# ziqin-h/GIVEPose

Measured on AMD Instinct MI355X. Metric: images/sec PoseNet fwd, bs=64 256x256 fp16, 1/2/4/8 MI355X; % MFMA roofline, higher is better.
Workload: dtype f16

## Files before the change

givepose_amd/_lib.py:

```python
import ctypes
import os
from ctypes import POINTER, Structure, c_char_p, c_double, c_float, c_int, c_long, c_void_p

_HERE = os.path.dirname(os.path.abspath(__file__))
LIB_PATH = os.environ.get("GP_LIB_PATH") or os.path.join(_HERE, "libgivepose_hip.so")

ABI_VERSION = 328
GP_F32, GP_F16, GP_F64 = 0, 1, 2
ACT_NONE, ACT_GELU, ACT_RELU, ACT_LRELU = 0, 1, 2, 3
EPI_NONE, EPI_GELU, EPI_RELU, EPI_LRELU, EPI_SCALE_RES, EPI_RES_RELU, EPI_LNFOLD_GELU = 0, 1, 2, 3, 4, 5, 6
ROT_6D, ROT_6D_Y, ROT_6D_Z, ROT_QUAT, ROT_EULER = 0, 1, 2, 3, 4
KC_GEMM, KC_DCNV3, KC_DWCONV_LN, KC_NORM, KC_ELEMENTWISE, KC_SMALL, KC_COUNT = 0, 1, 2, 3, 4, 5, 6
KC_NAMES = ["gemm", "dcnv3", "dwconv_ln", "norm", "elementwise", "small"]


class GemmDesc(Structure):
    _fields_ = [("X", c_void_p), ("W", c_void_p), ("bias", c_void_p), ("gamma", c_void_p), ("residual", c_void_p),
                ("C", c_void_p), ("workspace", c_void_p),
                ("M", c_int), ("N", c_int), ("K", c_int), ("ldx", c_int), ("ldc", c_int), ("ldres", c_int),
                ("epilogue", c_int), ("out_f32", c_int), ("splitk", c_int),
                ("B", c_int), ("H", c_int), ("Win", c_int), ("Cin", c_int), ("KH", c_int), ("KW", c_int),
                ("stride", c_int), ("pad", c_int), ("Ho", c_int), ("Wo", c_int), ("dtype", c_int),
                ("gn_partial", c_void_p), ("gn_groups", c_int), ("gn_hw", c_int), ("variant", c_int),
                ("ln_stats", c_void_p), ("ln_colsum", c_void_p), ("ln_nslab", c_int), ("ln_eps", c_float),
# ... 316 lines not shown


class RepackBnFold(Structure):
    _fields_ = [(n, c_void_p) for n in ("w", "b", "bn_w", "bn_b", "mean", "var", "w_out", "b_out")] + [
        ("w_numel", c_longlong), ("c_numel", c_longlong), ("C", c_int), ("K", c_int), ("eps", c_float), ("pad", c_int)]


class RepackMatFold(Structure):
    _fields_ = [(n, c_void_p) for n in ("A", "B", "add", "out32", "out64")] + [
        (n, c_longlong) for n in ("a_numel", "b_numel", "add_numel", "out32_numel", "out64_numel")] + [
        (n, c_int) for n in ("M", "N", "K", "a_rs", "b_rs", "ld32", "ld64", "b_f64", "level", "pad")]


class RepackInfo(Structure):
    _fields_ = [(n, c_longlong) for n in ("bytes", "off_chunks", "off_bn", "off_mat", "off_mchunks")] + [
        (n, c_int) for n in ("n_entries", "n_chunks", "n_bn", "n_bn_blocks", "n_mat", "n_mchunks0", "n_mchunks1", "pad")]


REPACK_PROTOTYPES = {
    "gpr_tables_bytes": ([POINTER(RepackEntry), c_int, POINTER(RepackBnFold), c_int, POINTER(RepackMatFold), c_int], c_longlong),
    "gpr_tables_upload": ([POINTER(RepackEntry), c_int, POINTER(RepackBnFold), c_int, POINTER(RepackMatFold), c_int, _P, _P, c_longlong,
                           POINTER(RepackInfo), _P], c_int),
    "gpr_repack": ([_P, POINTER(RepackInfo), _P], c_int),
}
GPR_CHUNK, GPR_REPACK_LAUNCHES, GPR_REPACK_LAUNCHES_F32, GPR_MAX_ENTRIES, GPR_MAX_DIMS = 4096, 4, 3, 65536, 4
GPR_KIND_F32, GPR_KIND_F16, GPR_KIND_SPLIT = 0, 1, 2

TRAINDATA_PROTOTYPES = {
    "gpt_crop_train": ([_P] * 21 + [c_int] * 7 + [_P], c_int),
    "gpt_mask_deform": ([_P] * 3 + [c_ulonglong, _P, c_int, c_int, _P], c_int),
}
GPT_MAX_PIXELS, GPT_TRAIN_BATCH_LAUNCHES = 65536, 2

_lib = None


class GivePoseHipError(RuntimeError):
    pass


def load():
    global _lib
    if _lib is not None:
        return _lib
    if not os.path.exists(LIB_PATH):
        raise GivePoseHipError(
            f"{LIB_PATH} not found: build it with `python -m givepose_amd.build` (hipcc --offload-arch=gfx950). "
            "There is no CPU or PyTorch fallback for the product path.")
    lib = ctypes.CDLL(LIB_PATH)
    for name, (argtypes, restype) in (list(PROTOTYPES.items()) + list(ALIGN_PROTOTYPES.items()) + list(LOSS_PROTOTYPES.items())
                                      + list(GRAD_PROTOTYPES.items()) + list(HEADGRAD_PROTOTYPES.items())
                                      + list(XYZGRAD_PROTOTYPES.items()) + list(XYZGRAD_BF16_PROTOTYPES.items()) + list(ENCGRAD_PROTOTYPES.items())
                                      + list(ENCGRAD_ORDERED_PROTOTYPES.items())
                                      + list(BBGRAD_PROTOTYPES.items()) + list(BBGRAD_BF16_PROTOTYPES.items()) + list(OPTIM_PROTOTYPES.items())
                                      + list(SIZEGRAD_PROTOTYPES.items()) + list(ACCUM_PROTOTYPES.items())
                                      + list(REPACK_PROTOTYPES.items()) + list(TRAINDATA_PROTOTYPES.items())
                                      + list(ADAM_PROTOTYPES.items())):
        fn = getattr(lib, name)
        fn.argtypes = argtypes
        fn.restype = restype
    if lib.gp_version() != ABI_VERSION:
        raise GivePoseHipError(f"{LIB_PATH}: ABI version {lib.gp_version()}, this package needs {ABI_VERSION}: rebuild with "
                               "`python -m givepose_amd.build`")
    _lib = lib
    return lib


def check(rc, what=""):
    if rc != 0:
        msg = load().gp_last_error()
        raise GivePoseHipError(f"{what} failed ({rc}): {msg.decode() if msg else ''}")


_capturing = 0


def capturing():
    return _capturing > 0
```

givepose_amd/build.py:

```python
import os
import subprocess
import sys

HERE = os.path.dirname(os.path.abspath(__file__))
CSRC = os.path.join(HERE, "csrc")
OBJ = os.path.join(HERE, "csrc", "build")
LIB = os.path.join(HERE, "libgivepose_hip.so")
SOURCES = ["runtime.hip", "gemm.hip", "mlp.hip", "dcnv3.hip", "dcnv3_any.hip", "norm.hip", "misc.hip", "scalenet.hip", "evalmap.hip", "align.hip", "loss.hip", "lossgrad.hip", "pnpgrad.hip", "xyzgrad.hip", "encgrad.hip", "encscatter.hip", "bbgrad.hip", "optim.hip", "sizegrad.hip", "accum.hip", "repack.hip", "traindata.hip", "adam.hip"]
HIPCC = os.environ.get("HIPCC", "/opt/rocm/bin/hipcc")
FLAGS = ["-O3", "--offload-arch=gfx950", "-fPIC", "-std=c++17", "-Wno-unused-value"]
if os.environ.get("GP_PACKED_FP32") != "1":
    FLAGS += ["-Xclang", "-target-feature", "-Xclang", "-packed-fp32-ops", "-Wno-unknown-warning-option"]
EXTRA = os.environ.get("GP_EXTRA_HIPCC_FLAGS", "").split()
TAG = os.environ.get("GP_BUILD_TAG", "")
if EXTRA and not TAG:
    raise RuntimeError("GP_EXTRA_HIPCC_FLAGS needs GP_BUILD_TAG: an investigation build must not overwrite the product library")
if TAG:
    OBJ = os.path.join(HERE, "csrc", "build", "tag_" + TAG)
    LIB = os.path.join(HERE, f"libgivepose_hip_{TAG}.so")
    FLAGS += EXTRA


def _newer(a, b):
    return not os.path.exists(b) or os.path.getmtime(a) > os.path.getmtime(b)


def build(force=False, verbose=True):
    os.makedirs(OBJ, exist_ok=True)
    deps = [os.path.join(CSRC, "common.hpp"), os.path.join(HERE, "..", "include", "givepose_hip.h"),
            os.path.join(HERE, "..", "include", "givepose_align.h"), os.path.join(CSRC, "align_math.hpp"),
            os.path.join(HERE, "..", "include", "givepose_loss.h"), os.path.join(HERE, "..", "include", "givepose_grad.h"),
            os.path.join(HERE, "..", "include", "givepose_headgrad.h"), os.path.join(HERE, "..", "include", "givepose_xyzgrad.h"),
            os.path.join(HERE, "..", "include", "givepose_encgrad.h"), os.path.join(HERE, "..", "include", "givepose_bbgrad.h"),
            os.path.join(HERE, "..", "include", "givepose_optim.h"), os.path.join(HERE, "..", "include", "givepose_sizegrad.h"),
            os.path.join(HERE, "..", "include", "givepose_accum.h"), os.path.join(HERE, "..", "include", "givepose_repack.h"),
            os.path.join(HERE, "..", "include", "givepose_traindata.h"), os.path.join(CSRC, "grad_gemm.hpp"), os.path.join(CSRC, "grad_gemm_bf16.hpp"),
            os.path.join(HERE, "..", "include", "givepose_bbgrad_bf16.h"), os.path.join(CSRC, "xyz_conv_prec.hpp"),
            os.path.join(HERE, "..", "include", "givepose_xyzgrad_bf16.h"),
            os.path.join(HERE, "..", "include", "givepose_encgrad_ordered.h"), os.path.join(CSRC, "encscatter.hpp"),
            os.path.join(HERE, "..", "include", "givepose_adam.h")]
    objs, procs = [], []
    for src in SOURCES:
        s, o = os.path.join(CSRC, src), os.path.join(OBJ, src.replace(".hip", ".o"))
        objs.append(o)
        if force or _newer(s, o) or any(_newer(d, o) for d in deps):
            if verbose:
                print("hipcc", src, flush=True)
            procs.append((src, subprocess.Popen([HIPCC, *FLAGS, "-c", s, "-o", o])))
    for src, p in procs:
        if p.wait() != 0:
            raise RuntimeError(f"hipcc failed on {src}")
    if force or procs or not os.path.exists(LIB) or any(_newer(o, LIB) for o in objs):
        subprocess.check_call([HIPCC, "--offload-arch=gfx950", "-shared", "-fPIC", "-o", LIB, *objs])
        if verbose:
            print("linked", LIB)
    return LIB


if __name__ == "__main__":
    build(force="--force" in sys.argv)
```

givepose_amd/config.py:

```python
from dataclasses import dataclass, field
from typing import Tuple


ROT_TYPES = {
    "allo_rot6d": (6, 0, True), "ego_rot6d": (6, 0, False), "allo_rot6d_sym": (6, 0, True), "allo_rot6d_x": (6, 0, True),
    "allo_rot6d_sym_y": (6, 1, True), "allo_rot6d_y": (6, 1, True), "allo_rot6d_z": (6, 2, True),
    "allo_quat": (4, 3, True), "ego_quat": (4, 3, False), "euler": (6, 4, False),
}
FLAT_OPS = {"flatten": 0, "avg": 1, "avg-max": 2, "avg-max-min": 3}


def validate(cfg):
    def one_of(name, allowed):
        v = getattr(cfg, name)
        if v not in allowed:
            raise ValueError(f"{name}={v!r}: expected one of {sorted(allowed)}")
    if cfg.mask_attention_type == "concat":
        raise NotImplementedError("mask_attention_type='concat': the reference builds ConvPnPNet(5, ...) and then feeds it 6 channels "
                                  "(PoseNet.py:140,162; conv_pnp_net.py:73,152), so it cannot run this mode either")
    one_of("mask_attention_type", ("none", "mul"))
    one_of("flat_op", FLAT_OPS)
    one_of("r_type", ROT_TYPES)
    one_of("nocsmap_encoder", ("conv", "att"))
    one_of("use_dcn", ("dcnv3", ""))
# ... 11 lines not shown
                                      "its (B, 64, 192) tokens (attention_pnp_net.py:90-106), so fc1 gets 64 columns where it expects "
                                      f"{192 * FLAT_OPS[cfg.flat_op]}; the reference cannot run it either")
        if cfg.mask_attention_type == "mul":
            raise NotImplementedError("pnp_head='att' with mask_attention_type='mul': AttentionPnPNet.forward takes no mask "
                                      "(attention_pnp_net.py:121)")
        if ROT_TYPES[cfg.r_type][0] != 6:
            raise NotImplementedError(f"pnp_head='att' with r_type={cfg.r_type!r}: AttentionPnPNet's fc_r is Linear(256, 6) whatever the "
                                      "rotation type (attention_pnp_net.py:72), and a quaternion needs 4 outputs")


@dataclass(frozen=True)
class PoseNetConfig:
    main_backbone: str = "convnext"
    img_size: int = 256
    out_res: int = 64
    mask_attention_type: str = "none"
    feat_ts: int = 128
    flat_op: str = "flatten"
    t_type: str = "site"
    size_head_out_dim: int = 3
    nocsmap_encoder: str = "conv"
    r_type: str = "allo_rot6d"
    use_dcn: str = "dcnv3"
    dataset: str = "CAMERA+Real"
    convnext_dims: Tuple[int, ...] = (128, 256, 512, 1024)
    convnext_depths: Tuple[int, ...] = (3, 3, 27, 3)
    fuse_mlp: bool = True
    fuse_mlp_min_batch: int = 16
    defer_ln: bool = False

    res_fp32: bool = False
    deconv_cols_f16: bool = True
    gnxyz16: bool = True
    fuse_mlp512: bool = False
    pnp_head: str = "conv"

    @property
    def rot_dim(self) -> int:
        return ROT_TYPES[self.r_type][0] if self.r_type in ROT_TYPES else (4 if "quat" in self.r_type else 6)

    @property
    def fc_in_dim(self) -> int:
        k = FLAT_OPS[self.flat_op]
        if self.pnp_head == "att":
            return 192 * (k or 64)
        return 128 * (k or 64)

    @property
    def feature_channel(self) -> int:
        return {"convnext": self.convnext_dims[-1], "resnet34": 512}[self.main_backbone]
```

givepose_amd/csrc/misc.hip:

```cpp
#include "common.hpp"

namespace {

__device__ __forceinline__ void store_T(half_t* p, float v) { *p = (half_t)v; }
__device__ __forceinline__ void store_T(float* p, float v) { *p = v; }

template <typename T>
__global__ __launch_bounds__(256) void stem_kernel(const float* __restrict__ img, const float* __restrict__ wt,
                                                   const float* __restrict__ bias, const float* __restrict__ lnw,
                                                   const float* __restrict__ lnb, T* __restrict__ out, int H,
                                                   int W, float eps, int PXB) {
    constexpr int C0 = 128;
    __shared__ __attribute__((aligned(16))) float in_s[12][256];
    const int Ho = H / 4, Wo = W / 4;
    const int tid = threadIdx.x, lane = tid & 63, wave = tid >> 6;
    const int nwb = Wo / PXB;
    const int wblk = blockIdx.x % nwb;
    const int ho = (blockIdx.x / nwb) % Ho;
    const int b = blockIdx.x / (nwb * Ho);
    const int wo0 = wblk * PXB;
    for (int i = tid; i < 12 * PXB * 4; i += 256) {
        const int row = i / (PXB * 4), col = i - row * (PXB * 4);
        const int c = row >> 2, kh = row & 3;
        in_s[row][col] = img[(((long)b * 3 + c) * H + (ho * 4 + kh)) * W + wo0 * 4 + col];
    }
    float2 wr[48];
#pragma unroll
    for (int k = 0; k < 48; ++k) wr[k] = *reinterpret_cast<const float2*>(wt + k * C0 + lane * 2);
    const float2 bv = *reinterpret_cast<const float2*>(bias + lane * 2);
    const float2 gw = *reinterpret_cast<const float2*>(lnw + lane * 2), gb = *reinterpret_cast<const float2*>(lnb + lane * 2);
    __syncthreads();
    const int ppw = PXB / 4;
    for (int q = 0; q < ppw; ++q) {
// ... 283 lines not shown
template <typename T, typename CT>
__global__ __launch_bounds__(256) void col2im_kernel(const CT* __restrict__ cols, T* __restrict__ out, int B,
                                                     int H, int W, int C) {
    constexpr int VEC = 16 / sizeof(CT);
    const int CV = C / VEC, Ho = 2 * H, Wo = 2 * W;
    const long idx = (long)blockIdx.x * 256 + threadIdx.x;
    if (idx >= (long)B * Ho * Wo * CV) return;
    const int cv = (int)(idx % CV);
    long t = idx / CV;
    const int ox = (int)(t % Wo); t /= Wo;
    const int oy = (int)(t % Ho);
    const long b = t / Ho;
    float a[VEC];
#pragma unroll
    for (int e = 0; e < VEC; ++e) a[e] = 0.f;
    for (int ky = 0; ky < 3; ++ky) {
        const int ty = oy + 1 - ky;
        if (ty < 0 || (ty & 1)) continue;
        const int i = ty >> 1;
        if (i >= H) continue;
        for (int kx = 0; kx < 3; ++kx) {
            const int tx = ox + 1 - kx;
            if (tx < 0 || (tx & 1)) continue;
            const int j = tx >> 1;
            if (j >= W) continue;
            const Vec16<CT> v = load16<CT>(cols + ((b * H + i) * W + j) * (9L * C) + (ky * 3 + kx) * C + cv * VEC);
#pragma unroll
            for (int e = 0; e < VEC; ++e) a[e] += v.get(e);
        }
    }
    T* o = out + ((b * Ho + oy) * Wo + ox) * C + cv * VEC;
#pragma unroll
    for (int e = 0; e < VEC; ++e) store_T(o + e, a[e]);
}

template <typename T>
__global__ __launch_bounds__(256) void xyz_out_kernel(const T* __restrict__ x, const float* __restrict__ w,
                                                      const float* __restrict__ bias, float* __restrict__ out_nchw,
                                                      float* __restrict__ out_nhwc4, long rows, int HW, int C) {
    constexpr int VEC = Vec16<T>::N;
    const int chunks = C / VEC;
    const int LPP = chunks < 64 ? chunks : 64;
    const int lane = threadIdx.x & 63;
    const int sub = lane / LPP, l = lane % LPP;
    const int ppw = 64 / LPP;
    const long wave_id = (long)blockIdx.x * 4 + (threadIdx.x >> 6);
    const long row = wave_id * ppw + sub;
    float a0 = 0.f, a1 = 0.f, a2 = 0.f;
    if (row < rows) {
        for (int c = l; c < chunks; c += LPP) {
            const Vec16<T> v = load16<T>(x + row * C + c * VEC);
#pragma unroll
            for (int e = 0; e < VEC; ++e) {
                const float f = v.get(e);
                const int ch = c * VEC + e;
                a0 += f * w[ch];
                a1 += f * w[C + ch];
                a2 += f * w[2 * C + ch];
            }
        }
    }
    a0 = group_sum(a0, LPP); a1 = group_sum(a1, LPP); a2 = group_sum(a2, LPP);
    if (row < rows && l == 0) {
        a0 += bias[0]; a1 += bias[1]; a2 += bias[2];
        const long b = row / HW, pix = row - b * HW;
        out_nchw[(b * 3 + 0) * HW + pix] = a0;
// ... 638 lines not shown
               "gp_crop_rois: null pointer");
    GP_REQUIRE(B > 0 && B <= 65535 && F > 0 && NM > 0 && H > 0 && W > 0 && S > 0 && R > 0 && R <= S, "gp_crop_rois: bad shape");
    hipStream_t s = (hipStream_t)stream;
    gp_timing_before(s, GP_KC_SMALL, 0.0, (double)B * (S * S * 4.0 * 4 + S * S * 4.0 + R * R * 8.0));
    hipLaunchKernelGGL(crop_rois_kernel, dim3(cdiv(S * S, 256), B), dim3(256), 0, s, frames, masks, frame_idx, mask_idx, inv_img,
                       inv_out, img_lut, xlut, ylut, roi_img, roi_mask, roi_coord_2d, H, W, S, R);
    GP_LAUNCH_CHECK("gp_crop_rois");
}

extern "C" int gp_pred_rt(const float* R, const float* t, const float* size, const float* scale, float* pred_rt,
                          float* pred_size, int B, void* stream) {
    GP_REQUIRE(R && t && size && pred_rt && pred_size && B > 0, "gp_pred_rt: bad argument");
    hipStream_t s = (hipStream_t)stream;
    gp_timing_before(s, GP_KC_SMALL, 0.0, (double)B * 35 * 4);
    hipLaunchKernelGGL(pred_rt_kernel, dim3(cdiv(B, 64)), dim3(64), 0, s, R, t, size, scale, pred_rt, pred_size, B);
    GP_LAUNCH_CHECK("gp_pred_rt");
}

extern "C" int gp_deconv_col2im(const void* cols, void* out, int B, int H, int W, int C, int dtype_in, void* stream) {
    const int dtype = dtype_in & ~GP_COLS_F16;
    const bool c16 = (dtype_in & GP_COLS_F16) != 0;
    GP_REQUIRE(cols && out && B > 0 && C % (c16 ? 8 : 4) == 0, "gp_deconv_col2im: bad argument");
    GP_DT_OK(dtype);
    GP_REQUIRE(!c16 || dtype == GP_F16, "gp_deconv_col2im: fp16 cols go with fp16 output");
    hipStream_t s = (hipStream_t)stream;
    const long total = (long)B * 4 * H * W * (C / (c16 ? 8 : 4));
    gp_timing_before(s, GP_KC_ELEMENTWISE, (double)B * H * W * 9 * C, (double)B * H * W * 9 * C * (c16 ? 2 : 4) + (double)B * 4 * H * W * C * (dtype == GP_F16 ? 2 : 4));
    if (c16) hipLaunchKernelGGL((col2im_kernel<half_t, half_t>), dim3(cdiv(total, 256)), dim3(256), 0, s, (const half_t*)cols, (half_t*)out, B, H, W, C);
    else if (dtype == GP_F16) hipLaunchKernelGGL((col2im_kernel<half_t, float>), dim3(cdiv(total, 256)), dim3(256), 0, s, (const float*)cols, (half_t*)out, B, H, W, C);
    else hipLaunchKernelGGL((col2im_kernel<float, float>), dim3(cdiv(total, 256)), dim3(256), 0, s, (const float*)cols, (float*)out, B, H, W, C);
    GP_LAUNCH_CHECK("gp_deconv_col2im");
}

extern "C" int gp_xyz_out_layer(const void* x, const float* w, const float* b, float* out_nchw, float* out_nhwc4,
                                int B, int HW, int C, int dtype, void* stream) {
    GP_REQUIRE(x && w && b && out_nchw && out_nhwc4 && B > 0, "gp_xyz_out_layer: bad argument");
    GP_DT_OK(dtype);
    const int esz = dtype == GP_F16 ? 2 : 4, vec = 16 / esz, chunks = C / vec;
    GP_REQUIRE(C % vec == 0 && (chunks & (chunks - 1)) == 0, "gp_xyz_out_layer: C=%d", C);
    const int LPP = chunks < 64 ? chunks : 64, ppw = 64 / LPP;
    const long rows = (long)B * HW;
    hipStream_t s = (hipStream_t)stream;
    gp_timing_before(s, GP_KC_SMALL, 6.0 * rows * C, (double)rows * C * esz + rows * 28.0);
    dim3 grid(cdiv(rows, 4L * ppw));
    if (dtype == GP_F16) hipLaunchKernelGGL(xyz_out_kernel<half_t>, grid, dim3(256), 0, s, (const half_t*)x, w, b, out_nchw, out_nhwc4, rows, HW, C);
    else hipLaunchKernelGGL(xyz_out_kernel<float>, grid, dim3(256), 0, s, (const float*)x, w, b, out_nchw, out_nhwc4, rows, HW, C);
    GP_LAUNCH_CHECK("gp_xyz_out_layer");
}

extern "C" int gp_pointwise_k3(const float* xyz4, const float* w, const float* b, void* y, long rows, int Cout,
                               int dtype, void* stream) {
    GP_REQUIRE(xyz4 && w && b && y && rows > 0, "gp_pointwise_k3: bad argument");
    GP_DT_OK(dtype);
    const int esz = dtype == GP_F16 ? 2 : 4, vec = 16 / esz;
    GP_REQUIRE(Cout % vec == 0 && 256 % (Cout / vec) == 0, "gp_pointwise_k3: Cout=%d", Cout);
    hipStream_t s = (hipStream_t)stream;
    const long total = cdiv(rows, (256 / (Cout / vec)) * 8) * 256;
    gp_timing_before(s, GP_KC_ELEMENTWISE, 6.0 * rows * Cout, rows * 16.0 + (double)rows * Cout * esz);
    gp_timing_label("pointwise_k3 rows%ld Cout%d", rows, Cout);
    if (dtype == GP_F16) hipLaunchKernelGGL(pointwise_k3_kernel<half_t>, dim3(cdiv(total, 256)), dim3(256), 0, s, xyz4, w, b, (half_t*)y, rows, Cout);
    else hipLaunchKernelGGL(pointwise_k3_kernel<float>, dim3(cdiv(total, 256)), dim3(256), 0, s, xyz4, w, b, (float*)y, rows, Cout);
    GP_LAUNCH_CHECK("gp_pointwise_k3");
}

template <int CIN>
static int launch_smallcin(const float* xyz4, const float* coord2d, const float* w, void* y, int B, int R, int Cout,
// ... 236 lines not shown
```

givepose_amd/ops.py:

```python
import ctypes
import os

import torch

from . import _lib
from ._lib import (ACT_GELU, ACT_LRELU, ACT_NONE, ACT_RELU, EPI_GELU, EPI_LNFOLD_GELU, EPI_LRELU, EPI_NONE, EPI_RELU, EPI_RES_RELU,
                   EPI_SCALE_RES, GP_F16, GP_F32, GP_F64, GemmDesc, check)

__all__ = ["dtype_code", "gemm", "conv2d_nhwc", "dcnv3_forward", "dcnv3_backward", "dcnv3_forward_into", "dcnv3_xyz_project", "convnext_stem", "dwconv_ln",
           "layernorm", "groupnorm", "upsample_bilinear2x", "deconv_col2im", "xyz_out_layer", "pointwise_k3",
           "pnp_conv1", "pnp_conv1_masked", "pool_mmm", "xyz_conv3x3_s2", "size_head", "pose_tail", "pose_tail_rt", "mask_resize_nearest"]


def _L():
    return _lib.load()


def _stream():
    return ctypes.c_void_p(torch.cuda.current_stream().cuda_stream)


def dtype_code(dt):
    if dt == torch.float16:
        return GP_F16
    if dt == torch.float32:
        return GP_F32
    raise TypeError(f"unsupported dtype {dt} (float16 / float32)")


def _ptr(t):
    return None if t is None else ctypes.c_void_p(t.data_ptr())


def _chk(t, name, dtype=None):
    if not t.is_cuda:
        raise RuntimeError(f"{name} must be a CUDA tensor")
    if dtype is not None and t.dtype != dtype:
        raise TypeError(f"{name}: expected {dtype}, got {t.dtype}")
    return t


def _contig(t, name):
    if not t.is_contiguous():
# ... 400 lines not shown
    check(_L().gp_groupnorm_apply(_ptr(x), _ptr(partial), _ptr(w), _ptr(b), _ptr(out), B, HW, C, G, eps, act,
                                  C if ldy is None else ldy, HW // rows if fused_stats else 0, _planes_code(x, out_planes, out), _stream()),
          "gp_groupnorm_apply")
    return out


def groupnorm_upsample2x(x, w, b, out, G, act, partial, eps=1e-5, rows=64):
    B, H, W_, C = x.shape
    check(_L().gp_groupnorm_upsample2x(_ptr(_contig(x, "x")), _ptr(partial), _ptr(w), _ptr(b), _ptr(out), B, H, W_, C, G, eps, act,
                                       H * W_ // rows, dtype_code(x.dtype), _stream()), "gp_groupnorm_upsample2x")
    return out


def groupnorm_apply_xyz(x, w, b, out_w, out_b, out_nchw, out_nhwc4, G, act, partial, eps=1e-5, rows=64, packed16=False):
    B, HW, C = x.shape
    check(_L().gp_groupnorm_apply_xyz(_ptr(_contig(x, "x")), _ptr(partial), _ptr(w), _ptr(b), _ptr(out_w), _ptr(out_b),
                                      _ptr(out_nchw), _ptr(out_nhwc4), B, HW, C, G, eps, act | (0x100 if packed16 else 0), HW // rows, dtype_code(x.dtype),
                                      _stream()), "gp_groupnorm_apply_xyz")


def upsample_bilinear2x(x, out, out_planes=False):
    B, H, W_, C = x.shape
    check(_L().gp_upsample_bilinear2x(_ptr(_contig(x, "x")), _ptr(out), B, H, W_, C, _planes_code(x, out_planes, out), _stream()),
          "gp_upsample_bilinear2x")
    return out


def deconv_col2im(cols, out, B, H, W_, C):
    code = dtype_code(out.dtype) | (0x400 if cols.dtype == torch.float16 else 0)
    check(_L().gp_deconv_col2im(_ptr(cols), _ptr(out), B, H, W_, C, code, _stream()), "gp_deconv_col2im")
    return out


def xyz_out_layer(x, w, b, out_nchw, out_nhwc4):
    B, HW, C = x.shape
    check(_L().gp_xyz_out_layer(_ptr(_contig(x, "x")), _ptr(w), _ptr(b), _ptr(out_nchw), _ptr(out_nhwc4), B, HW, C,
                                dtype_code(x.dtype), _stream()), "gp_xyz_out_layer")


def pointwise_k3(xyz4, w, b, out):
    rows = xyz4.shape[0]
    check(_L().gp_pointwise_k3(_ptr(xyz4), _ptr(w), _ptr(b), _ptr(out), rows, w.shape[0], dtype_code(out.dtype), _stream()),
          "gp_pointwise_k3")
    return out


def dcnv3_xyz_project(xyz4, om, m, bias, out, gn, mask_col=72, mask_is_logits=True):
    _contig(_chk(xyz4, "xyz4"), "xyz4"), _contig(_chk(om, "om"), "om"), _contig(_chk(out, "out"), "out")
    rows = out.shape[0]
    if xyz4.dtype != torch.float32 or om.dtype != torch.float32 or m.dtype != torch.float32 or bias.dtype != torch.float32:
        raise TypeError("dcnv3_xyz_project: xyz4, om, m and bias are float32")
    if tuple(m.shape) != (256, 16) or bias.numel() != 256 or out.shape[1] != 256 or om.shape[0] < rows or xyz4.shape[0] < (rows + 1023) // 1024 * 4096:
        raise RuntimeError("dcnv3_xyz_project: shapes")
    if gn[0].numel() < (rows + 1023) // 1024 * 32 * 32 * 2:
        raise RuntimeError("dcnv3_xyz_project: the gn_partial buffer is too small for 32 chunks of 32 groups per crop")
    check(_L().gp_dcnv3_xyz_project(_ptr(xyz4), _ptr(om), _ptr(_contig(m, "m")), _ptr(bias), _ptr(out), _ptr(gn[0]), rows, 64, 64, 3, 2, 1, 1, 4,
                                    om.shape[1], mask_col, 1 if mask_is_logits else 0, gn[1], gn[2], gn[3], dtype_code(out.dtype), _stream()),
          "gp_dcnv3_xyz_project")
    return out


def pnp_conv1(xyz4, coord2d, w, out, B, R):
    check(_L().gp_pnp_conv1(_ptr(xyz4), _ptr(_contig(coord2d, "coord2d")), _ptr(w), _ptr(out), B, R, w.shape[1],
                            dtype_code(out.dtype), _stream()), "gp_pnp_conv1")
    return out

# ... 65 lines not shown
```

givepose_amd/posenet.py:

```python
import ctypes
import functools
import os
from collections import OrderedDict

import numpy as np
import torch
import torch.nn as nn

from . import _lib, ops, synth
from ._lib import (ACT_GELU, ACT_RELU, EPI_GELU, EPI_LNFOLD_GELU, EPI_LRELU, EPI_NONE, EPI_SCALE_RES)
from .config import FLAT_OPS, ROT_TYPES, PoseNetConfig, validate

OM_LD = 128


def enc0_xyz_pack(sd, prefix="nocs_encoder.features.0.", dtype=torch.float32):
    f64 = lambda k: sd[prefix + k].detach().to(device="cpu", dtype=torch.float64)
    cw, cb = f64("conv.weight").reshape(256, -1), f64("conv.bias")
    iw, ib = f64("dcnv3.input_proj.weight"), f64("dcnv3.input_proj.bias")
    ow, ob = f64("dcnv3.output_proj.weight"), f64("dcnv3.output_proj.bias")
    fold = torch.cat([iw @ cw, (iw @ cb + ib)[:, None]], 1)
    m = torch.cat([ow[:, 64 * g:64 * g + 64] @ fold[64 * g:64 * g + 64] for g in range(4)], 1)
    return m.to(dtype).contiguous(), ob.to(dtype).contiguous()

# ... 384 lines not shown
                buf[f"dsn{s}"] = e(B, h * 2, h * 2, dims[s - 1])
        buf["cols"] = e(B * 64, 9 * 256) if (T == torch.float16 and cfg.deconv_cols_f16 and os.environ.get("GP_DECONV_COLS_F32") != "1") else f(B * 64, 9 * 256)
        for r in (16, 32, 64):
            buf[f"ya{r}"], buf[f"yb{r}"] = e(B, r, r, 256), e(B, r, r, 256)
        chunks = max(ops.groupnorm_chunks(B, r * r) for r in (8, 16, 32, 64))
        buf["gn_partial"], buf["size_scratch"] = f(B * max(chunks, R * R // 16) * 32 * 2), f(B * (cfg.feat_ts + (512 if cfg.main_backbone == "resnet34" else cfg.convnext_dims[-1])))
        buf["nocs_nchw"], buf["nocs_nhwc4"] = f(B, 3, R, R), f(B * R * R, 4)
        buf["ivfc_nchw"], buf["ivfc_nhwc4"] = f(B, 3, R, R), f(B * R * R, 4)
        buf["mask_out"], buf["size"] = f(B, 1, R, R), f(B, 3)
        enc0_xyz = "enc0.xyz_m" in self._packed and os.environ.get("GP_ENC0_XYZ") != "0"
        for li, r in enumerate((64, 32, 16)):
            buf[f"e_in{li}"], buf[f"e_x1{li}"] = e(B, r, r, 256), e(B * r * r // 4, 256)
            buf[f"e_om{li}"] = f(B * r * r // 4, OM_LD)
            buf[f"e_o{li}"] = e(B, r // 2, r // 2, 256)
            if li > 0 or not enc0_xyz:
                buf[f"e_proj{li}"], buf[f"e_g{li}"] = e(B, r, r, 256), e(B, r // 2, r // 2, 256)
        if cfg.nocsmap_encoder == "att":
            buf["a_patch"], buf["a_x"], buf["a_h"] = e(B * 64, 192), e(B * 64, 256), e(B * 64, 256)
            buf["a_qkv"], buf["a_att"], buf["a_mlp"] = e(B * 64, 768), e(B * 64, 256), e(B * 64, 1024)
            buf["a_pos"] = self._packed["att.pos"].to(T).repeat(B, 1).contiguous()
        buf["feat_cat"] = e(B, 8, 8, 512)
        if cfg.pnp_head == "att":
            buf["p_patch"], buf["p_x"], buf["p_h"] = e(B * 64, 320), e(B * 64, 192), e(B * 64, 192)
            buf["p_qkv"], buf["p_att"], buf["p_mlp"], buf["p_flat"] = e(B * 64, 576), e(B * 64, 192), e(B * 64, 768), e(B * 64, 192)
            buf["p_pos"] = self._packed["apn.pos"].to(T).repeat(B, 1).contiguous()
        else:
            buf["p0"], buf["p1"], buf["p2"] = e(B, 32, 32, 128), e(B, 16, 16, 128), e(B, 8, 8, 128)
        buf["fc1"] = e(B, 2048)
        buf["hh"], buf["hz"] = f(B, 256), f(B, 256)
        if FLAT_OPS[cfg.flat_op]:
            buf["pooled"] = e(B, 128 * FLAT_OPS[cfg.flat_op])
        buf["pred_rot"], buf["pred_t"], buf["rot_allo"], buf["rot_ego"], buf["trans"] = f(B, cfg.rot_dim), f(B, 3), f(B, 9), f(B, 9), f(B, 3)
        buf["rot6d"] = buf["pred_rot"] if cfg.rot_dim == 6 else None
        plan = {"buf": buf, "graph": None, "warm": False, "ragged": bool(ragged), "enc0_xyz": enc0_xyz}
        if ragged:
            buf["grp"] = torch.arange(B, dtype=torch.int32, device=device)
            buf["grp_host"] = torch.arange(B, dtype=torch.int32).pin_memory()
            for k in ("roi_img", "roi_mask", "roi_coord_2d", "bbox_center", "mean_size"):
                buf[k].zero_()
            buf["roi_wh"].fill_(1.0)
            buf["resize_ratio"].fill_(1.0)
            buf["cam_K"].copy_(torch.eye(3, device=device).expand(B, 3, 3))
        self._plans[key] = plan
        self._evict_plans(key)
        return plan

    def _gn(self, x, w, b, act, buf, G=32, out=None, ldy=None, fused=False, out_planes=False, rows=64):
        B = x.shape[0]
        C = x.shape[-1]
        xv = x.view(B, -1, C)
        ops.groupnorm(xv, w, b, xv if out is None else out, G, act, buf["gn_partial"], ldy=ldy, fused_stats=fused, out_planes=out_planes, rows=rows)

    def _gnrows(self, M, N, K, hw):
        if self.split_gemm or self.compute_dtype != torch.float16 or os.environ.get("GP_GN_ROWS64") == "1":
            return 64
        return ops.gemm_gn_rows(M, N, K, hw)

    @staticmethod
    def _gnarg(buf, hw, rows=64):
        B = buf["mask_out"].shape[0]
        if B * (hw // rows) * 32 * 2 > buf["gn_partial"].numel():
            raise RuntimeError(f"fused GroupNorm statistics: {hw // rows} chunks of {rows} rows per image do not fit the plan's gn_partial buffer")
        return (buf["gn_partial"], 32, hw, rows)

    def _xyz_head(self, W, head, feat2d, B, buf, out_nchw, out_nhwc4):
        pl = self.split_gemm
        ops.gemm(feat2d, W[head + ".deconv_w"], buf["cols"], prefetch=W[f"{head}.c3_w"])
        y = ops.deconv_col2im(buf["cols"], buf["ya16"], B, 8, 8, 256)
        if pl:
            self._gn(y, W[head + ".gn0_w"], W[head + ".gn0_b"], ACT_GELU, buf, out=buf["yb16"].view(B, -1, 256), out_planes=True)
            y = buf["yb16"]
        else:
            self._gn(y, W[head + ".gn0_w"], W[head + ".gn0_b"], ACT_GELU, buf)
        cur, r = y, 16
        rows = {rr: self._gnrows(B * rr * rr, 256, 2304, rr * rr) for rr in (16, 32, 64)}
        fuse_up = FUSE_GN_UPSAMPLE and not pl and y.dtype == torch.float16
        for i in (3, 4, 6, 7, 9, 10):
            if i in (6, 9):
                r *= 2
                if fuse_up:
                    cur = ops.groupnorm_upsample2x(cur, W[f"{head}.c{i - 2}_gw"], W[f"{head}.c{i - 2}_gb"], buf[f"ya{r}"], 32, ACT_GELU,
                                                   buf["gn_partial"], rows=rows[r // 2])
                else:
                    cur = ops.upsample_bilinear2x(cur, buf[f"ya{r}"], out_planes=pl)
            dst = buf[f"yb{r}"] if cur is buf[f"ya{r}"] else buf[f"ya{r}"]
            nxt = {3: 4, 4: 6, 6: 7, 7: 9, 9: 10}.get(i)
            ops.conv2d_nhwc(cur, W[f"{head}.c{i}_w"], 3, 3, 1, 1, out=dst, gn=self._gnarg(buf, r * r, rows[r]),
                            prefetch=W[f"{head}.c{nxt}_w"] if nxt else None, x_planes=pl)
            if i == 10:
                ops.groupnorm_apply_xyz(dst.view(B, r * r, 256), W[f"{head}.c{i}_gw"], W[f"{head}.c{i}_gb"], W[head + ".out_w"],
                                        W[head + ".out_b"], out_nchw, out_nhwc4, 32, ACT_GELU, buf["gn_partial"], rows=rows[r],
                                        packed16=self.cfg.gnxyz16 and dst.dtype == torch.float16 and os.environ.get("GP_GNXYZ16") != "0")
            elif fuse_up and i in (4, 7):
                pass
            elif pl and i not in (4, 7):
                self._gn(dst, W[f"{head}.c{i}_gw"], W[f"{head}.c{i}_gb"], ACT_GELU, buf, fused=True, out=cur.view(B, -1, 256), out_planes=True, rows=rows[r])
                dst = cur
            else:
                self._gn(dst, W[f"{head}.c{i}_gw"], W[f"{head}.c{i}_gb"], ACT_GELU, buf, fused=True, rows=rows[r])
            cur = dst

    def _resnet34(self, W, buf):
        from ._lib import EPI_RELU, EPI_RES_RELU
        s = ops.resnet_stem(buf["roi_img"], W["rs.stem_w"], W["rs.stem_b"], buf["rs_stem"])
        x = ops.maxpool3x3s2(s, buf["rs1a"])
        for li, (planes, blocks, stride) in enumerate(synth.RESNET34_LAYERS, 1):
# ... 30 lines not shown
        for s, (d, n) in enumerate(zip(dims, depths)):
            if s > 0:
                t = ops.layernorm(x, W[f"ds{s}.ln_w"], W[f"ds{s}.ln_b"], buf[f"dsn{s}"], out_planes=self.split_gemm)
                x = ops.conv2d_nhwc(t, W[f"ds{s}.w"], 2, 2, 2, 0, out=buf[f"x{s}"], bias=W[f"ds{s}.b"], x_planes=self.split_gemm,
                                    out16=buf.get(f"x{s}h"))
            x2d = x.view(-1, d)
            xh = buf.get(f"x{s}h")
            xin = x if xh is None else xh
            for b in range(n):
                q = f"s{s}b{b}."
                if (q + "fc1_wg") in W and x2d.shape[0] % 256 == 0 and x.shape[1] % 4 == 0 and x.shape[2] % 16 == 0:
                    t = ops.dwconv7_raw_stats(x, W[q + "dw_w"], W[q + "dw_b"], buf[f"t{s}"], buf["ln_stats"])
                    ops.gemm(t.view(-1, d), W[q + "fc1_wg"], buf[f"h{s}"], bias=W[q + "fc1_cb"], epilogue=EPI_LNFOLD_GELU,
                             ln=(buf["ln_stats"], W[q + "fc1_cs"], d // 128, 1e-6))
                    ops.gemm(buf[f"h{s}"], W[q + "fc2_w"], x2d, bias=W[q + "fc2_b"], epilogue=EPI_SCALE_RES,
                             gamma=W[q + "gamma"], residual=x2d)
                    continue
                t = ops.dwconv_ln(xin, W[q + "dw_w"], W[q + "dw_b"], W[q + "ln_w"], W[q + "ln_b"], buf[f"t{s}"], 7, out_planes=self.split_gemm)
                if (q + "fc2_wp") in W and x2d.shape[0] % 256 == 0 and B >= cfg.fuse_mlp_min_batch and (d != 512 or x2d.shape[0] >= 32768):
                    ops.convnext_mlp(t.view(-1, d), W[q + "fc1_w"], W[q + "fc1_b"], W[q + "fc2_wp"], W[q + "fc2_b"],
                                     W[q + "gamma"], x2d, x2d)
                    continue
                pl = self.split_gemm
                ops.gemm(t.view(-1, d), W[q + "fc1_w"], buf[f"h{s}"], bias=W[q + "fc1_b"], epilogue=EPI_GELU, prefetch=W[q + "fc2_w"],
                         x_planes=pl, out_planes=pl)
                ops.gemm(buf[f"h{s}"], W[q + "fc2_w"], x2d, bias=W[q + "fc2_b"], epilogue=EPI_SCALE_RES,
                         gamma=W[q + "gamma"], residual=x2d, x_planes=pl, out16=None if xh is None else xh.view(-1, d),
                         prefetch=W.get(f"ds{s + 1}.w") if b == n - 1 else None)
        if cfg.main_backbone == "convnext":
            feat = x
        fc = dims[-1]
        feat2d = feat.view(B * 64, fc)
        ops.size_head(feat.view(B, 64, fc), W["size.w1"], W["size.b1"], W["size.w2"], W["size.b2"], buf["mean_size"], buf["size"], buf["size_scratch"])
        self._xyz_head(W, "xyz_nocs_head", feat2d, B, buf, buf["nocs_nchw"], buf["nocs_nhwc4"])
        self._seq_encoder(B, plan)
        cat2d = buf["feat_cat"].view(B * 64, 512)
        ops.gemm(feat2d, W["red.w"], cat2d, bias=W["red.b"], ldc=512)
        self._xyz_head(W, "xyz_deform_head", cat2d, B, buf, buf["ivfc_nchw"], buf["ivfc_nhwc4"])
        self._seq_pnp(B, plan)

    def _seq_encoder(self, B, plan, only_layer=None, weights_of=None):
        W, buf, cfg = self._packed, plan["buf"], self.cfg
        cat2d = buf["feat_cat"].view(B * 64, 512)
        prev = None
        if cfg.nocsmap_encoder == "att":
            x = buf["a_x"]
            ops.patchify_xyz(buf["nocs_nhwc4"], buf["a_patch"], B, cfg.out_res, 8)
            ops.gemm(buf["a_patch"], W["att.pe_w"], x, bias=W["att.pe_b"], epilogue=EPI_SCALE_RES, gamma=W["att.ones"],
                     residual=buf["a_pos"])
            for i in range(3):
                q = f"att{i}."
                h = ops.layernorm(x, W[q + "norm1_w"], W[q + "norm1_b"], buf["a_h"], eps=1e-5)
                ops.gemm(h, W[q + "qkv_w"], buf["a_qkv"])
                ops.attention64(buf["a_qkv"], buf["a_att"], B, 8)
                ops.gemm(buf["a_att"], W[q + "proj_w"], x, bias=W[q + "proj_b"], epilogue=EPI_SCALE_RES, gamma=W["att.ones"], residual=x)
                h = ops.layernorm(x, W[q + "norm2_w"], W[q + "norm2_b"], buf["a_h"], eps=1e-5)
                ops.gemm(h, W[q + "fc1_w"], buf["a_mlp"], bias=W[q + "fc1_b"], epilogue=EPI_GELU)
                ops.gemm(buf["a_mlp"], W[q + "fc2_w"], x, bias=W[q + "fc2_b"], epilogue=EPI_SCALE_RES, gamma=W["att.ones"], residual=x)
            ops.layernorm(x, W["att.norm_w"], W["att.norm_b"], cat2d[:, 256:], eps=1e-5, ldy=512)
        for li, r in enumerate((64, 32, 16) if cfg.nocsmap_encoder == "conv" else ()):
            q = f"enc{li}."
            ro = r // 2
            if only_layer is not None:
                if li != only_layer:
                    continue
                prev = buf[f"e_o{li - 1}"]
                if weights_of is not None:
                    q = f"enc{weights_of}."
            if cfg.use_dcn == "dcnv3":
                xin = buf[f"e_in{li}"]
                xyz0 = li == 0 and plan.get("enc0_xyz") and only_layer is None
# ... 186 lines not shown
                        _lib._capturing -= 1
                        ge = ctypes.c_void_p()
                        rc = lib.gp_graph_end(sp, ctypes.byref(ge))
                    _lib.check(rc, "gp_graph_end")
                    plan["graph"] = ge
                _lib.check(lib.gp_graph_launch(plan["graph"], sp), "gp_graph_launch")
            else:
                self._launch_all(B, plan)
                plan["warm"] = True
        if run_stream is not cur and wait:
            cur.wait_stream(run_stream)
        n = n_real
        feat = buf.get(f"x{len(self.cfg.convnext_dims) - 1}")
        return {"rot": buf["rot_ego"].view(B, 3, 3)[:n], "trans": buf["trans"][:n], "size": buf["size"][:n], "mask": buf["mask_out"][:n],
                "nocs_coor": buf["nocs_nchw"][:n], "ivfc_coor": buf["ivfc_nchw"][:n], "rot6d": None if buf["rot6d"] is None else buf["rot6d"][:n],
                "pred_rot": buf["pred_rot"][:n], "pred_t": buf["pred_t"][:n],
                "rot_allo": buf["rot_allo"].view(B, 3, 3)[:n], "feat": None if feat is None else feat[:n],
                "feat_cat": buf["feat_cat"][:n]}

    def _module_plan(self, B, device):
        device = torch.device(device)
        _lib.load()
        if self._packed is None:
            self._pack(device)
        return self._plan(B, device, 0)

    @torch.no_grad()
    def run_xyz_head(self, head, feat_nchw, device="cuda"):
        B, C = feat_nchw.shape[:2]
        plan = self._module_plan(B, device)
        buf = plan["buf"]
        x = feat_nchw.to(device).permute(0, 2, 3, 1).reshape(B * 64, C).to(self.compute_dtype).contiguous()
        key = "nocs" if head == "xyz_nocs_head" else "ivfc"
        self._xyz_head(self._packed, head, x, B, buf, buf[key + "_nchw"], buf[key + "_nhwc4"])
        return buf[key + "_nchw"].clone()

    @torch.no_grad()
    def run_map_encoder(self, coor_nchw, device="cuda"):
        B = coor_nchw.shape[0]
        plan = self._module_plan(B, device)
        buf = plan["buf"]
        buf["nocs_nhwc4"].zero_()
        buf["nocs_nhwc4"][:, :3] = coor_nchw.to(device).float().permute(0, 2, 3, 1).reshape(-1, 3)
        self._seq_encoder(B, plan)
        return buf["feat_cat"].view(B, 8, 8, 512)[..., 256:].permute(0, 3, 1, 2).float().contiguous()

    @torch.no_grad()
    def run_dcnv3_c(self, layer, x_nchw, device="cuda", weights_of=None):
        assert self.cfg.use_dcn == "dcnv3" and layer in (1, 2) and weights_of in (None, 1, 2)
        B = x_nchw.shape[0]
        plan = self._module_plan(B, device)
        buf = plan["buf"]
        buf[f"e_o{layer - 1}"].copy_(x_nchw.to(device).permute(0, 2, 3, 1).to(self.compute_dtype))
        self._seq_encoder(B, plan, only_layer=layer, weights_of=weights_of)
        return buf[f"e_o{layer}"].permute(0, 3, 1, 2).float().contiguous()

    @torch.no_grad()
    def run_pnp(self, x_nchw, data, device="cuda", mask=None):
        B = x_nchw.shape[0]
        if self.cfg.mask_attention_type == "mul" and mask is None:
            raise ValueError("run_pnp: mask_attention_type='mul' needs the (B,1,64,64) mask")
        plan = self._module_plan(B, device)
        buf = plan["buf"]
        if mask is not None:
            buf["mask_out"].copy_(mask.reshape(buf["mask_out"].shape))
        for k in ("cam_K", "roi_wh", "bbox_center", "resize_ratio"):
            buf[k].copy_(data[k].reshape(buf[k].shape))
# ... 373 lines not shown
```

Baseline: 12730.

## Fuse deconv col2im with GroupNorm and GELU in xyz heads

Adds a HIP kernel that performs the transposed-conv col2im gather for the first 16x16 map of each xyz head and computes GroupNorm statistics, affine and GELU inside one workgroup per image and channel slab. Each thread keeps its gathered pixels in registers for the two-pass mean and variance. This removes the intermediate ya16 write/read and the separate GroupNorm statistics and apply launches. The path is on by default for fp16, non-split plans and has an environment switch. The cost is a per-thread register footprint of GS half8 vectors and fixed shape requirements: a 256-pixel output map and 8 channels per group.

```diff
diff --git a/givepose_amd/_lib.py b/givepose_amd/_lib.py
--- a/givepose_amd/_lib.py
+++ b/givepose_amd/_lib.py
@@ -372,6 +372,10 @@
 }
 GPT_MAX_PIXELS, GPT_TRAIN_BATCH_LAUNCHES = 65536, 2
 
+FUSED_PROTOTYPES = {
+    "gpfu_deconv_col2im_gn": ([_P] * 4 + [c_int] * 5 + [c_float] + [c_int] * 2 + [_P], c_int),
+}
+
 _lib = None
 
 
@@ -395,7 +399,7 @@
                                       + list(BBGRAD_PROTOTYPES.items()) + list(BBGRAD_BF16_PROTOTYPES.items()) + list(OPTIM_PROTOTYPES.items())
                                       + list(SIZEGRAD_PROTOTYPES.items()) + list(ACCUM_PROTOTYPES.items())
                                       + list(REPACK_PROTOTYPES.items()) + list(TRAINDATA_PROTOTYPES.items())
-                                      + list(ADAM_PROTOTYPES.items())):
+                                      + list(ADAM_PROTOTYPES.items()) + list(FUSED_PROTOTYPES.items())):
         fn = getattr(lib, name)
         fn.argtypes = argtypes
         fn.restype = restype
diff --git a/givepose_amd/build.py b/givepose_amd/build.py
--- a/givepose_amd/build.py
+++ b/givepose_amd/build.py
@@ -38,7 +38,7 @@
             os.path.join(HERE, "..", "include", "givepose_bbgrad_bf16.h"), os.path.join(CSRC, "xyz_conv_prec.hpp"),
             os.path.join(HERE, "..", "include", "givepose_xyzgrad_bf16.h"),
             os.path.join(HERE, "..", "include", "givepose_encgrad_ordered.h"), os.path.join(CSRC, "encscatter.hpp"),
-            os.path.join(HERE, "..", "include", "givepose_adam.h")]
+            os.path.join(HERE, "..", "include", "givepose_adam.h"), os.path.join(HERE, "..", "include", "givepose_fused.h")]
     objs, procs = [], []
     for src in SOURCES:
         s, o = os.path.join(CSRC, src), os.path.join(OBJ, src.replace(".hip", ".o"))
diff --git a/givepose_amd/config.py b/givepose_amd/config.py
--- a/givepose_amd/config.py
+++ b/givepose_amd/config.py
@@ -67,6 +67,7 @@
     res_fp32: bool = False
     deconv_cols_f16: bool = True
     gnxyz16: bool = True
+    col2im_gn_min_batch: int = 1
     fuse_mlp512: bool = False
     pnp_head: str = "conv"
 
diff --git a/givepose_amd/csrc/misc.hip b/givepose_amd/csrc/misc.hip
--- a/givepose_amd/csrc/misc.hip
+++ b/givepose_amd/csrc/misc.hip
@@ -1,4 +1,5 @@
 #include "common.hpp"
+#include "../../include/givepose_fused.h"
 
 namespace {
 
@@ -348,6 +349,116 @@
     T* o = out + ((b * Ho + oy) * Wo + ox) * C + cv * VEC;
 #pragma unroll
     for (int e = 0; e < VEC; ++e) store_T(o + e, a[e]);
+}
+
+template <typename CT, int GS>
+__global__ __launch_bounds__(256) void col2im_gn_kernel(const CT* __restrict__ cols, const float* __restrict__ w,
+                                                        const float* __restrict__ bb, half_t* __restrict__ out, int H, int W,
+                                                        int C, float eps, int act) {
+    constexpr int PPS = 256 / GS;
+    __shared__ float red_s[4][GS], red_q[4][GS];
+    const int Ho = 2 * H, Wo = 2 * W, nslab = C / (8 * GS);
+    const long b = blockIdx.x / nslab;
+    const int slab = blockIdx.x % nslab;
+    const int v = threadIdx.x % GS, pl = threadIdx.x / GS, wave = threadIdx.x >> 6;
+    const int c0 = (slab * GS + v) * 8;
+    half8 x[GS];
+    float s = 0.f;
+#pragma unroll
+    for (int u = 0; u < GS; ++u) {
+        const int p = u * PPS + pl, oy = p / Wo, ox = p % Wo;
+        const int ky0 = (oy & 1) ? 0 : 1, kx0 = (ox & 1) ? 0 : 1;
+        const int i0 = (oy + 1 - ky0) >> 1, j0 = (ox + 1 - kx0) >> 1, i1 = (oy - 1) >> 1, j1 = (ox - 1) >> 1;
+        const bool vy[2] = {i0 < H, (oy & 1) != 0}, vx[2] = {j0 < W, (ox & 1) != 0};
+        const int ii[2] = {i0, i1}, jj[2] = {j0, j1}, kyy[2] = {ky0, 2}, kxx[2] = {kx0, 2};
+        float a[8];
+#pragma unroll
+        for (int e = 0; e < 8; ++e) a[e] = 0.f;
+        if constexpr (sizeof(CT) == 2) {
+            half8 t[4];
+#pragma unroll
+            for (int k = 0; k < 4; ++k) {
+                const int ty = k >> 1, tx = k & 1;
+#pragma unroll
+                for (int e = 0; e < 8; ++e) t[k][e] = (half_t)0.f;
+                if (vy[ty] && vx[tx]) t[k] = *reinterpret_cast<const half8*>(cols + ((b * H + ii[ty]) * W + jj[tx]) * (9L * C) + (kyy[ty] * 3 + kxx[tx]) * C + c0);
+            }
+#pragma unroll
+            for (int k = 0; k < 4; ++k)
+#pragma unroll
+                for (int e = 0; e < 8; ++e) a[e] += (float)t[k][e];
+        } else {
+            f32x4 t[4][2];
+#pragma unroll
+            for (int k = 0; k < 4; ++k) {
+                const int ty = k >> 1, tx = k & 1;
+                t[k][0] = t[k][1] = f32x4{0.f, 0.f, 0.f, 0.f};
+                if (vy[ty] && vx[tx]) {
+                    const CT* src = cols + ((b * H + ii[ty]) * W + jj[tx]) * (9L * C) + (kyy[ty] * 3 + kxx[tx]) * C + c0;
+                    t[k][0] = *reinterpret_cast<const f32x4*>(src);
+                    t[k][1] = *reinterpret_cast<const f32x4*>(src + 4);
+                }
+            }
+#pragma unroll
+            for (int k = 0; k < 4; ++k)
+#pragma unroll
+                for (int e = 0; e < 4; ++e) { a[e] += t[k][0][e]; a[e + 4] += t[k][1][e]; }
+        }
+#pragma unroll
+        for (int e = 0; e < 8; ++e) {
+            x[u][e] = (half_t)a[e];
+            s += (float)x[u][e];
+        }
+    }
+    const float inv_n = 1.0f / (float)(Ho * Wo * 8);
+#pragma unroll
+    for (int d = GS; d < 64; d <<= 1) s += __shfl_xor(s, d, 64);
+    if ((threadIdx.x & 63) < GS) red_s[wave][v] = s;
+    __syncthreads();
+    const float mean = (((red_s[0][v] + red_s[1][v]) + red_s[2][v]) + red_s[3][v]) * inv_n;
+    float q = 0.f;
+#pragma unroll
+    for (int u = 0; u < GS; ++u)
+#pragma unroll
+        for (int e = 0; e < 8; ++e) {
+            const float d = (float)x[u][e] - mean;
+            q = fmaf(d, d, q);
+        }
+#pragma unroll
+    for (int d = GS; d < 64; d <<= 1) q += __shfl_xor(q, d, 64);
+    if ((threadIdx.x & 63) < GS) red_q[wave][v] = q;
+    __syncthreads();
+    const float var = (((red_q[0][v] + red_q[1][v]) + red_q[2][v]) + red_q[3][v]) * inv_n;
+    const float rstd = 1.0f / sqrtf(var + eps);
+    float sc[8], sh[8];
+    {
+        const f32x4 w0 = *reinterpret_cast<const f32x4*>(w + c0), w1 = *reinterpret_cast<const f32x4*>(w + c0 + 4);
+        const f32x4 b0 = *reinterpret_cast<const f32x4*>(bb + c0), b1 = *reinterpret_cast<const f32x4*>(bb + c0 + 4);
+#pragma unroll
+        for (int e = 0; e < 4; ++e) {
+            sc[e] = rstd * w0[e];
+            sc[e + 4] = rstd * w1[e];
+            sh[e] = __fmaf_rn(-mean, sc[e], b0[e]);
+            sh[e + 4] = __fmaf_rn(-mean, sc[e + 4], b1[e]);
+        }
+    }
+#pragma unroll
+    for (int u = 0; u < GS; ++u) {
+        const int p = u * PPS + pl;
+        half8 o;
+        if (act == GP_ACT_GELU) {
+#pragma unroll
+            for (int e = 0; e < 8; e += 2) {
+                const f32x2 g = gelu_poly2(f32x2{__fmaf_rn((float)x[u][e], sc[e], sh[e]), __fmaf_rn((float)x[u][e + 1], sc[e + 1], sh[e + 1])});
+                o[e] = (half_t)g[0];
+                o[e + 1] = (half_t)g[1];
+            }
+        } else {
+#pragma unroll
+            for (int e = 0; e < 8; ++e) o[e] = (half_t)apply_act(__fmaf_rn((float)x[u][e], sc[e], sh[e]), act);
+        }
+        *reinterpret_cast<half8*>(out + (b * Ho * Wo + p) * C + c0) = o;
+    }
 }
 
 template <typename T>
@@ -1052,6 +1163,24 @@
     GP_LAUNCH_CHECK("gp_deconv_col2im");
 }
 
+extern "C" int gpfu_deconv_col2im_gn(const void* cols, const float* w, const float* b, void* out, int B, int H, int W, int C, int G,
+                                   float eps, int act, int dtype_in, void* stream) {
+    const int dtype = dtype_in & ~GP_COLS_F16;
+    const bool c16 = (dtype_in & GP_COLS_F16) != 0;
+    constexpr int GS = 4;
+    GP_REQUIRE(cols && w && b && out && B > 0, "gpfu_deconv_col2im_gn: bad argument");
+    GP_REQUIRE(dtype == GP_F16, "gpfu_deconv_col2im_gn: fp16 output only (the fp32 modes keep gp_deconv_col2im + gp_groupnorm_*)");
+    GP_REQUIRE(H > 0 && W > 0 && 4 * H * W == 256, "gpfu_deconv_col2im_gn: a workgroup holds a 256-pixel output map, got %d x %d", 2 * H, 2 * W);
+    GP_REQUIRE(G > 0 && C == 8 * G && C % (8 * GS) == 0, "gpfu_deconv_col2im_gn: unsupported C=%d G=%d (8 channels per group, C %% %d == 0)", C, G, 8 * GS);
+    GP_REQUIRE((long)B * (C / (8 * GS)) <= 0x7fffffffL, "gpfu_deconv_col2im_gn: B=%d too large", B);
+    hipStream_t s = (hipStream_t)stream;
+    gp_timing_before(s, GP_KC_NORM, (double)B * H * W * 9 * C + 10.0 * B * 4 * H * W * C, (double)B * H * W * 9 * C * (c16 ? 2 : 4) + (double)B * 4 * H * W * C * 2);
+    const dim3 grid(B * (C / (8 * GS)));
+    if (c16) hipLaunchKernelGGL((col2im_gn_kernel<half_t, GS>), grid, dim3(256), 0, s, (const half_t*)cols, w, b, (half_t*)out, H, W, C, eps, act);
+    else hipLaunchKernelGGL((col2im_gn_kernel<float, GS>), grid, dim3(256), 0, s, (const float*)cols, w, b, (half_t*)out, H, W, C, eps, act);
+    GP_LAUNCH_CHECK("gpfu_deconv_col2im_gn");
+}
+
 extern "C" int gp_xyz_out_layer(const void* x, const float* w, const float* b, float* out_nchw, float* out_nhwc4,
                                 int B, int HW, int C, int dtype, void* stream) {
     GP_REQUIRE(x && w && b && out_nchw && out_nhwc4 && B > 0, "gp_xyz_out_layer: bad argument");
diff --git a/givepose_amd/ops.py b/givepose_amd/ops.py
--- a/givepose_amd/ops.py
+++ b/givepose_amd/ops.py
@@ -8,7 +8,7 @@
                    EPI_SCALE_RES, GP_F16, GP_F32, GP_F64, GemmDesc, check)
 
 __all__ = ["dtype_code", "gemm", "conv2d_nhwc", "dcnv3_forward", "dcnv3_backward", "dcnv3_forward_into", "dcnv3_xyz_project", "convnext_stem", "dwconv_ln",
-           "layernorm", "groupnorm", "upsample_bilinear2x", "deconv_col2im", "xyz_out_layer", "pointwise_k3",
+           "layernorm", "groupnorm", "upsample_bilinear2x", "deconv_col2im", "deconv_col2im_gn", "xyz_out_layer", "pointwise_k3",
            "pnp_conv1", "pnp_conv1_masked", "pool_mmm", "xyz_conv3x3_s2", "size_head", "pose_tail", "pose_tail_rt", "mask_resize_nearest"]
 
 
@@ -475,6 +475,15 @@
     return out
 
 
+def deconv_col2im_gn(cols, w, b, out, B, H, W_, C, G, act, eps=1e-5):
+    if out.dtype != torch.float16:
+        raise TypeError(f"deconv_col2im_gn writes fp16, got {out.dtype}")
+    code = GP_F16 | (0x400 if cols.dtype == torch.float16 else 0)
+    check(_L().gpfu_deconv_col2im_gn(_ptr(_contig(cols, "cols")), _ptr(w), _ptr(b), _ptr(_contig(out, "out")), B, H, W_, C, G, eps, act, code,
+                                     _stream()), "gpfu_deconv_col2im_gn")
+    return out
+
+
 def xyz_out_layer(x, w, b, out_nchw, out_nhwc4):
     B, HW, C = x.shape
     check(_L().gp_xyz_out_layer(_ptr(_contig(x, "x")), _ptr(w), _ptr(b), _ptr(out_nchw), _ptr(out_nhwc4), B, HW, C,
diff --git a/givepose_amd/posenet.py b/givepose_amd/posenet.py
--- a/givepose_amd/posenet.py
+++ b/givepose_amd/posenet.py
@@ -440,7 +440,8 @@
             buf["pooled"] = e(B, 128 * FLAT_OPS[cfg.flat_op])
         buf["pred_rot"], buf["pred_t"], buf["rot_allo"], buf["rot_ego"], buf["trans"] = f(B, cfg.rot_dim), f(B, 3), f(B, 9), f(B, 9), f(B, 3)
         buf["rot6d"] = buf["pred_rot"] if cfg.rot_dim == 6 else None
-        plan = {"buf": buf, "graph": None, "warm": False, "ragged": bool(ragged), "enc0_xyz": enc0_xyz}
+        col2im_gn = (T == torch.float16 and not self.split_gemm and 0 < cfg.col2im_gn_min_batch <= B and os.environ.get("GP_COL2IM_GN") != "0")
+        plan = {"buf": buf, "graph": None, "warm": False, "ragged": bool(ragged), "enc0_xyz": enc0_xyz, "col2im_gn": col2im_gn}
         if ragged:
             buf["grp"] = torch.arange(B, dtype=torch.int32, device=device)
             buf["grp_host"] = torch.arange(B, dtype=torch.int32).pin_memory()
@@ -471,15 +472,18 @@
             raise RuntimeError(f"fused GroupNorm statistics: {hw // rows} chunks of {rows} rows per image do not fit the plan's gn_partial buffer")
         return (buf["gn_partial"], 32, hw, rows)
 
-    def _xyz_head(self, W, head, feat2d, B, buf, out_nchw, out_nhwc4):
+    def _xyz_head(self, W, head, feat2d, B, buf, out_nchw, out_nhwc4, col2im_gn=False):
         pl = self.split_gemm
         ops.gemm(feat2d, W[head + ".deconv_w"], buf["cols"], prefetch=W[f"{head}.c3_w"])
-        y = ops.deconv_col2im(buf["cols"], buf["ya16"], B, 8, 8, 256)
-        if pl:
-            self._gn(y, W[head + ".gn0_w"], W[head + ".gn0_b"], ACT_GELU, buf, out=buf["yb16"].view(B, -1, 256), out_planes=True)
-            y = buf["yb16"]
+        if col2im_gn:
+            y = ops.deconv_col2im_gn(buf["cols"], W[head + ".gn0_w"], W[head + ".gn0_b"], buf["ya16"], B, 8, 8, 256, 32, ACT_GELU)
         else:
-            self._gn(y, W[head + ".gn0_w"], W[head + ".gn0_b"], ACT_GELU, buf)
+            y = ops.deconv_col2im(buf["cols"], buf["ya16"], B, 8, 8, 256)
+            if pl:
+                self._gn(y, W[head + ".gn0_w"], W[head + ".gn0_b"], ACT_GELU, buf, out=buf["yb16"].view(B, -1, 256), out_planes=True)
+                y = buf["yb16"]
+            else:
+                self._gn(y, W[head + ".gn0_w"], W[head + ".gn0_b"], ACT_GELU, buf)
         cur, r = y, 16
         rows = {rr: self._gnrows(B * rr * rr, 256, 2304, rr * rr) for rr in (16, 32, 64)}
         fuse_up = FUSE_GN_UPSAMPLE and not pl and y.dtype == torch.float16
@@ -576,11 +580,11 @@
         fc = dims[-1]
         feat2d = feat.view(B * 64, fc)
         ops.size_head(feat.view(B, 64, fc), W["size.w1"], W["size.b1"], W["size.w2"], W["size.b2"], buf["mean_size"], buf["size"], buf["size_scratch"])
-        self._xyz_head(W, "xyz_nocs_head", feat2d, B, buf, buf["nocs_nchw"], buf["nocs_nhwc4"])
+        self._xyz_head(W, "xyz_nocs_head", feat2d, B, buf, buf["nocs_nchw"], buf["nocs_nhwc4"], plan["col2im_gn"])
         self._seq_encoder(B, plan)
         cat2d = buf["feat_cat"].view(B * 64, 512)
         ops.gemm(feat2d, W["red.w"], cat2d, bias=W["red.b"], ldc=512)
-        self._xyz_head(W, "xyz_deform_head", cat2d, B, buf, buf["ivfc_nchw"], buf["ivfc_nhwc4"])
+        self._xyz_head(W, "xyz_deform_head", cat2d, B, buf, buf["ivfc_nchw"], buf["ivfc_nhwc4"], plan["col2im_gn"])
         self._seq_pnp(B, plan)
 
     def _seq_encoder(self, B, plan, only_layer=None, weights_of=None):
@@ -833,7 +837,7 @@
         buf = plan["buf"]
         x = feat_nchw.to(device).permute(0, 2, 3, 1).reshape(B * 64, C).to(self.compute_dtype).contiguous()
         key = "nocs" if head == "xyz_nocs_head" else "ivfc"
-        self._xyz_head(self._packed, head, x, B, buf, buf[key + "_nchw"], buf[key + "_nhwc4"])
+        self._xyz_head(self._packed, head, x, B, buf, buf[key + "_nchw"], buf[key + "_nhwc4"], plan["col2im_gn"])
         return buf[key + "_nchw"].clone()
 
     @torch.no_grad()
diff --git a/include/givepose_fused.h b/include/givepose_fused.h
--- /dev/null
+++ b/include/givepose_fused.h
@@ -0,0 +1,16 @@
+#ifndef GIVEPOSE_FUSED_H
+#define GIVEPOSE_FUSED_H
+
+#include "givepose_hip.h"
+
+#ifdef __cplusplus
+extern "C" {
+#endif
+
+int gpfu_deconv_col2im_gn(const void* cols, const float* w, const float* b, void* out, int B, int H, int W, int C, int G,
+                          float eps, int act, int dtype, void* stream);
+
+#ifdef __cplusplus
+}
+#endif
+#endif
```

Result: no change. 12730 (-0.0%).
